# Developer-Zer0/GIF-synthesis-with-Discrete-Diffusion

Hardware: NVIDIA B200
Metric: reverse_step_token_updates_per_sec (higher is better)
Workload: dtype f32

## Files before the change

gif-synthesis-with-discrete-diffusion_b200/csrc/d3pm_ptx.cuh:

```cuda
#pragma once

#include <cuda_runtime.h>
#include <stdint.h>

namespace d3pm {

__device__ __forceinline__ uint32_t smem_u32(const void* p) { return static_cast<uint32_t>(__cvta_generic_to_shared(p)); }

__device__ __forceinline__ void mbar_init(unsigned long long* bar, uint32_t count) {
  asm volatile("mbarrier.init.shared::cta.b64 [%0], %1;" ::"r"(smem_u32(bar)), "r"(count) : "memory");
}
__device__ __forceinline__ void fence_mbarrier_init() { asm volatile("fence.mbarrier_init.release.cluster;" ::: "memory"); }
__device__ __forceinline__ void mbar_expect_tx(unsigned long long* bar, uint32_t bytes) {
  asm volatile("mbarrier.arrive.expect_tx.shared::cta.b64 _, [%0], %1;" ::"r"(smem_u32(bar)), "r"(bytes) : "memory");
}
__device__ __forceinline__ void mbar_arrive(unsigned long long* bar) {
  asm volatile("mbarrier.arrive.shared::cta.b64 _, [%0];" ::"r"(smem_u32(bar)) : "memory");
}
__device__ __forceinline__ void mbar_arrive_remote(unsigned long long* bar, uint32_t cta) {
  uint32_t r;
  asm volatile("mapa.shared::cluster.u32 %0, %1, %2;" : "=r"(r) : "r"(smem_u32(bar)), "r"(cta));
  asm volatile("mbarrier.arrive.release.cluster.shared::cluster.b64 _, [%0];" ::"r"(r) : "memory");
}
__device__ __forceinline__ bool mbar_test(unsigned long long* bar, uint32_t parity) {
  uint32_t done;
  asm volatile(
      "{\n\t.reg .pred p;\n\t"
      "mbarrier.test_wait.parity.shared::cta.b64 p, [%1], %2;\n\t"
      "selp.u32 %0, 1, 0, p;\n\t}"
      : "=r"(done)
      : "r"(smem_u32(bar)), "r"(parity)
      : "memory");
  return done != 0;
}
__device__ __forceinline__ void mbar_wait(unsigned long long* bar, uint32_t parity) {
  asm volatile(
      "{\n\t.reg .pred p;\n\t"
      "WAIT_%=:\n\t"
      "mbarrier.try_wait.parity.shared::cta.b64 p, [%0], %1, %2;\n\t"
      "@p bra DONE_%=;\n\t"
      "bra WAIT_%=;\n\t"
      "DONE_%=:\n\t}"
      ::"r"(smem_u32(bar)), "r"(parity), "r"(0x989680)
      : "memory");
}
__device__ __forceinline__ void mbar_wait_spin(unsigned long long* bar, uint32_t parity) {
  const uint32_t addr = smem_u32(bar);
  uint32_t done;
  do {
    asm volatile(
        "{\n\t.reg .pred p;\n\t"
        "mbarrier.try_wait.parity.shared::cta.b64 p, [%1], %2;\n\t"
        "selp.u32 %0, 1, 0, p;\n\t}"
        : "=r"(done)
        : "r"(addr), "r"(parity)
        : "memory");
  } while (!done);
}
__device__ __forceinline__ void mbar_wait_cluster(unsigned long long* bar, uint32_t parity) {
  asm volatile(
      "{\n\t.reg .pred p;\n\t"
      "WAIT_%=:\n\t"
      "mbarrier.try_wait.parity.acquire.cluster.shared::cta.b64 p, [%0], %1, %2;\n\t"
      "@p bra DONE_%=;\n\t"
      "bra WAIT_%=;\n\t"
      "DONE_%=:\n\t}"
      ::"r"(smem_u32(bar)), "r"(parity), "r"(0x989680)
      : "memory");
}

__device__ __forceinline__ void tma_load(void* dst, const void* src, uint32_t bytes, unsigned long long* bar) {
  asm volatile(
      "cp.async.bulk.shared::cluster.global.mbarrier::complete_tx::bytes [%0], [%1], %2, [%3];"
      ::"r"(smem_u32(dst)), "l"(src), "r"(bytes), "r"(smem_u32(bar))
      : "memory");
}
__device__ __forceinline__ void fence_proxy_async() { asm volatile("fence.proxy.async.shared::cta;" ::: "memory"); }

__device__ __forceinline__ void tc_fence_before() { asm volatile("tcgen05.fence::before_thread_sync;" ::: "memory"); }
__device__ __forceinline__ void tc_fence_after() { asm volatile("tcgen05.fence::after_thread_sync;" ::: "memory"); }
__device__ __forceinline__ void tc_commit(unsigned long long* bar) {
  asm volatile("tcgen05.commit.cta_group::1.mbarrier::arrive::one.shared::cluster.b64 [%0];" ::"r"(smem_u32(bar)) : "memory");
}
__device__ __forceinline__ void tc_commit_pair(unsigned long long* bar) {
  asm volatile("tcgen05.commit.cta_group::2.mbarrier::arrive::one.shared::cluster.multicast::cluster.b64 [%0], %1;" ::"r"(smem_u32(bar)),
               "h"(static_cast<unsigned short>(3))
               : "memory");
}
constexpr uint32_t idesc_tf32(int M, int N) {
  return (1u << 4) | (2u << 7) | (2u << 10) | ((static_cast<uint32_t>(N) >> 3) << 17) | ((static_cast<uint32_t>(M) >> 4) << 24);
}
__device__ __forceinline__ void tc_mma_tf32(uint32_t d_tmem, uint64_t a_desc, uint64_t b_desc, uint32_t idesc, uint32_t accumulate) {
  asm volatile(
      "{\n\t.reg .pred p;\n\t"
      "setp.ne.b32 p, %4, 0;\n\t"
      "tcgen05.mma.cta_group::1.kind::tf32 [%0], %1, %2, %3, p;\n\t}"
      ::"r"(d_tmem), "l"(a_desc), "l"(b_desc), "r"(idesc), "r"(accumulate)
      : "memory");
}
__device__ __forceinline__ void tc_mma_tf32_pair(uint32_t d_tmem, uint64_t a_desc, uint64_t b_desc, uint32_t idesc, uint32_t accumulate) {
  asm volatile(
      "{\n\t.reg .pred p;\n\t"
      "setp.ne.b32 p, %4, 0;\n\t"
      "tcgen05.mma.cta_group::2.kind::tf32 [%0], %1, %2, %3, p;\n\t}"
      ::"r"(d_tmem), "l"(a_desc), "l"(b_desc), "r"(idesc), "r"(accumulate)
      : "memory");
}
__device__ __forceinline__ uint64_t smem_desc(uint32_t addr) {
  return static_cast<uint64_t>((addr >> 4) & 0x3fffu) | (static_cast<uint64_t>(1024 >> 4) << 32) | (1ull << 46) | (2ull << 61);
}

template <int CTAS, int NCOLS>
__device__ __forceinline__ void tmem_alloc(uint32_t* slot) {
  static_assert(CTAS == 1 || CTAS == 2, "cta_group::1 or ::2");
  if constexpr (CTAS == 2)
    asm volatile("tcgen05.alloc.cta_group::2.sync.aligned.shared::cta.b32 [%0], %1;" ::"r"(smem_u32(slot)), "n"(NCOLS) : "memory");
  else
    asm volatile("tcgen05.alloc.cta_group::1.sync.aligned.shared::cta.b32 [%0], %1;" ::"r"(smem_u32(slot)), "n"(NCOLS) : "memory");
}
template <int CTAS>
__device__ __forceinline__ void tmem_relinquish() {
  static_assert(CTAS == 1 || CTAS == 2, "cta_group::1 or ::2");
  if constexpr (CTAS == 2) asm volatile("tcgen05.relinquish_alloc_permit.cta_group::2.sync.aligned;" ::: "memory");
  else asm volatile("tcgen05.relinquish_alloc_permit.cta_group::1.sync.aligned;" ::: "memory");
}
template <int CTAS, int NCOLS>
__device__ __forceinline__ void tmem_dealloc(uint32_t taddr) {
  static_assert(CTAS == 1 || CTAS == 2, "cta_group::1 or ::2");
  if constexpr (CTAS == 2) asm volatile("tcgen05.dealloc.cta_group::2.sync.aligned.b32 %0, %1;" ::"r"(taddr), "n"(NCOLS) : "memory");
  else asm volatile("tcgen05.dealloc.cta_group::1.sync.aligned.b32 %0, %1;" ::"r"(taddr), "n"(NCOLS) : "memory");
}
__device__ __forceinline__ void tmem_ld16(uint32_t taddr, uint32_t (&v)[16]) {
  asm volatile(
      "tcgen05.ld.sync.aligned.32x32b.x16.b32 "
      "{%0, %1, %2, %3, %4, %5, %6, %7, %8, %9, %10, %11, %12, %13, %14, %15}, [%16];"
      : "=r"(v[0]), "=r"(v[1]), "=r"(v[2]), "=r"(v[3]), "=r"(v[4]), "=r"(v[5]), "=r"(v[6]), "=r"(v[7]), "=r"(v[8]),
        "=r"(v[9]), "=r"(v[10]), "=r"(v[11]), "=r"(v[12]), "=r"(v[13]), "=r"(v[14]), "=r"(v[15])
      : "r"(taddr)
      : "memory");
}
__device__ __forceinline__ void tmem_ld32(uint32_t taddr, uint32_t (&v)[32]) {
  asm volatile(
      "tcgen05.ld.sync.aligned.32x32b.x32.b32 "
      "{%0, %1, %2, %3, %4, %5, %6, %7, %8, %9, %10, %11, %12, %13, %14, %15, "
      "%16, %17, %18, %19, %20, %21, %22, %23, %24, %25, %26, %27, %28, %29, %30, %31}, [%32];"
      : "=r"(v[0]), "=r"(v[1]), "=r"(v[2]), "=r"(v[3]), "=r"(v[4]), "=r"(v[5]), "=r"(v[6]), "=r"(v[7]), "=r"(v[8]),
        "=r"(v[9]), "=r"(v[10]), "=r"(v[11]), "=r"(v[12]), "=r"(v[13]), "=r"(v[14]), "=r"(v[15]), "=r"(v[16]),
        "=r"(v[17]), "=r"(v[18]), "=r"(v[19]), "=r"(v[20]), "=r"(v[21]), "=r"(v[22]), "=r"(v[23]), "=r"(v[24]),
        "=r"(v[25]), "=r"(v[26]), "=r"(v[27]), "=r"(v[28]), "=r"(v[29]), "=r"(v[30]), "=r"(v[31])
      : "r"(taddr)
      : "memory");
}
__device__ __forceinline__ void tmem_ld_wait() { asm volatile("tcgen05.wait::ld.sync.aligned;" ::: "memory"); }

__device__ __forceinline__ uint32_t cluster_ctarank() {
  uint32_t r;
  asm volatile("mov.u32 %0, %%cluster_ctarank;" : "=r"(r));
  return r;
}
__device__ __forceinline__ void cluster_sync() {
  asm volatile("barrier.cluster.arrive.release;" ::: "memory");
  asm volatile("barrier.cluster.wait.acquire;" ::: "memory");
}

}
```

gif-synthesis-with-discrete-diffusion_b200/csrc/d3pm_step_stream.cuh:

```cuda
#pragma once

#include <type_traits>

#include "d3pm_host.h"
#include "d3pm_ptx.cuh"
#include "d3pm_step_rows.cuh"
#include "d3pm_stream.cuh"

namespace d3pm {

constexpr int kCandPerRow = 30;
constexpr float kStreamThin = 8.0f;
constexpr float kRedoThin = 16.0f;
struct RowInfo {
  float A, Bc, Pj, PK, accept;
  uint32_t j;
  int32_t rel;
  int32_t pad;
};

template <int NP, int CPT, bool HAS_U>
struct StreamShape {
  static_assert(CPT == 8 || (CPT == 16 && !HAS_U), "64 classes per thread only fit in registers without the second tensor");
  static constexpr int K = 1024 * NP;
  static constexpr int GT = 256 * NP / CPT;
  static constexpr int NW = GT / 32;
  static constexpr int NG = kStreamThreads / GT;
  static constexpr int SB = 128 / NG;
  static constexpr int RC = 8192 / NG;
  static constexpr int PS = 128 / GT;
  static constexpr int NCALL = CPT / 2;
  static_assert(GT >= 32 && GT <= 128 && NG <= 16, "unsupported group shape");
};

template <int NP, int CPT, bool HAS_U>
struct __align__(128) GroupSmem {
  using Sh = StreamShape<NP, CPT, HAS_U>;
  float c[1024 * NP];
  float u[HAS_U ? 1024 * NP : 4];
  alignas(16) float red[3][6 * 4];
  unsigned long long full;
  unsigned long long keys[4];
  uint32_t redo_cnt;
  uint32_t pad;
  RowInfo info[Sh::SB];
  uint32_t cand_cnt[Sh::SB];
  uint32_t cand_k[Sh::SB][kCandPerRow];
  float cand_p[Sh::SB][kCandPerRow];
  int32_t redo[Sh::RC];
};

template <int NW, int NV, typename Sync>
__device__ __forceinline__ void stream_max_sum(float (&m)[NV], float (&s)[NV], float* scratch, Sync sync) {
  const int lane = threadIdx.x & 31, warp = (threadIdx.x >> 5) & (NW - 1);
#pragma unroll
  for (int v = 0; v < NV; ++v) {
    const float mw = warp_max(m[v]);
    const float mw2 = to_log2_units(mw);
    const float sw = warp_sum(s[v] * ex2(to_log2_units(m[v]) - mw2));
    if (NW == 1) {
      m[v] = mw, s[v] = sw;
    } else if (lane == 0) {
      scratch[(3 * v) * 4 + warp] = mw;
      scratch[(3 * v + 1) * 4 + warp] = mw2;
      scratch[(3 * v + 2) * 4 + warp] = sw;
    }
  }
  sync();
  if constexpr (NW > 1) {
#pragma unroll
  for (int v = 0; v < NV; ++v) {
    const float4 mw = lds_warps<NW>(scratch + (3 * v) * 4, -CUDART_INF_F), mw2 = lds_warps<NW>(scratch + (3 * v + 1) * 4, 0.f);
    const float4 sw = lds_warps<NW>(scratch + (3 * v + 2) * 4, 0.f);
    if (NW == 4) {
      const float M = fmaxf(fmaxf(mw.x, mw.y), fmaxf(mw.z, mw.w));
      const float M2 = to_log2_units(M);
      m[v] = M;
      s[v] = fmaf(sw.x, ex2(mw2.x - M2), fmaf(sw.y, ex2(mw2.y - M2), fmaf(sw.z, ex2(mw2.z - M2), sw.w * ex2(mw2.w - M2))));
    } else {
      const float M = fmaxf(mw.x, mw.y);
      const float M2 = to_log2_units(M);
      m[v] = M;
      s[v] = fmaf(sw.x, ex2(mw2.x - M2), sw.y * ex2(mw2.y - M2));
    }
  }
  }
}

template <int NW, int NV, typename Sync>
__device__ __forceinline__ void stream_max(float* mx, float* scratch, Sync sync) {
  const int lane = threadIdx.x & 31, warp = (threadIdx.x >> 5) & (NW - 1);
#pragma unroll
  for (int v = 0; v < NV; ++v) {
    const float a = warp_max(mx[v]);
    if (NW == 1) mx[v] = a;
    else if (lane == 0) scratch[v * 4 + warp] = a;
  }
  sync();
  if constexpr (NW > 1) {
#pragma unroll
  for (int v = 0; v < NV; ++v) {
    const float4 a = lds_warps<NW>(scratch + v * 4, -CUDART_INF_F);
    mx[v] = fmaxf(fmaxf(a.x, a.y), fmaxf(a.z, a.w));
  }
  }
}

template <int NW, int NV, typename Sync>
__device__ __forceinline__ void stream_sum(float (&s)[NV], float* scratch, Sync sync) {
  const int lane = threadIdx.x & 31, warp = (threadIdx.x >> 5) & (NW - 1);
#pragma unroll
  for (int v = 0; v < NV; ++v) {
    const float sw = warp_sum(s[v]);
    if (NW == 1) s[v] = sw;
    else if (lane == 0) scratch[v * 4 + warp] = sw;
  }
  sync();
  if constexpr (NW > 1) {
#pragma unroll
  for (int v = 0; v < NV; ++v) {
    const float4 a = lds_warps<NW>(scratch + v * 4, 0.f);
    s[v] = (a.x + a.y) + (a.z + a.w);
  }
  }
}

template <int NW, typename Sync>
__device__ __forceinline__ unsigned long long stream_max_u64(unsigned long long key, unsigned long long* scratch, Sync sync) {
  const int lane = threadIdx.x & 31, warp = (threadIdx.x >> 5) & (NW - 1);
  key = warp_max_u64(key);
  if (NW == 1) {
    sync();
    return key;
  }
  if (lane == 0) scratch[warp] = key;
  sync();
  unsigned long long best = scratch[0];
#pragma unroll
  for (int w = 1; w < NW; ++w) best = scratch[w] > best ? scratch[w] : best;
  return best;
}

template <int NP, int CPT, bool HAS_U>
__device__ __noinline__ void score_batch(GroupSmem<NP, CPT, HAS_U>& S, int nslots, const ParamNoiseStream& rng, const StepParams& p, int G,
                                         int first_row) {
  using Sh = StreamShape<NP, CPT, HAS_U>;
  constexpr uint32_t K = 1024u * NP;
  const int lane = threadIdx.x & 31, warp = (threadIdx.x >> 5) & (Sh::NW - 1);
  const int sub = lane & 15;
  for (int slot = 2 * warp + (lane >> 4); slot - (lane >> 4) < nslots; slot += 2 * Sh::NW) {
    unsigned long long key = 0ull;
    float lp = 0.f;
    const bool live = slot < nslots;
    RowInfo ri;
    ri.accept = 0.f, ri.rel = 0;
    uint32_t cnt = 0;
    if (live) {
      ri = S.info[slot];
      cnt = S.cand_cnt[slot];
      const uint32_t n = cnt < static_cast<uint32_t>(kCandPerRow) ? cnt : static_cast<uint32_t>(kCandPerRow);
      const uint64_t grow = static_cast<uint64_t>(p.row_offset + (first_row + ri.rel * G));
      for (uint32_t item = static_cast<uint32_t>(sub); item < n + 2u; item += 16u) {
        uint32_t k = 0;
        float P = 0.f;
        bool have = false;
        if (item < n) {
          k = S.cand_k[slot][item];
          const float pe = fminf(fmaxf(S.cand_p[slot][item], kPFloor), 1.0f);
          P = fmaf(pe, ri.A, ri.Bc);
          have = (k != ri.j);
        } else if (item == n) {
          k = K, P = ri.PK, have = true;
        } else if (ri.j != K) {
          k = ri.j, P = ri.Pj, have = true;
        }
        if (have) {
          const float lpk = log_prob_clamped(P);
          const float sc = lpk + gumbel_from_uniform(uniform_from_draw(rng.draw(k, grow)));
          const unsigned long long kk = pack_key(sc, k);
          if (kk > key) key = kk, lp = lpk;
        }
      }
    }
    const unsigned long long mine = key;
#pragma unroll
    for (int o = 8; o > 0; o >>= 1) {
      const unsigned long long other = __shfl_xor_sync(0xffffffffu, key, o);
      key = other > key ? other : key;
    }
    const bool accepted = live && cnt <= static_cast<uint32_t>(kCandPerRow) && key_score(key) >= ri.accept;
    if (live && sub == 0) {
      if (accepted) {
        p.x_prev[first_row + ri.rel * G] = key_class(key);
      } else {
        S.redo[atomicAdd(&S.redo_cnt, 1u)] = ri.rel;
      }
      S.cand_cnt[slot] = 0;
    }
    if (p.winner_post != nullptr && accepted && mine == key && mine != 0ull) p.winner_post[first_row + ri.rel * G] = lp;
  }
}

template <int NP, int CPT, bool HAS_U, bool RECON, int LD = D3PM_LOGITS_F32>
__global__ void __launch_bounds__(kStreamThreads, 1) step_stream_kernel(const __grid_constant__ StepParams p) {
  extern __shared__ __align__(128) unsigned char smem_raw[];
  using Sh = StreamShape<NP, CPT, HAS_U>;
  using Smem = GroupSmem<NP, CPT, HAS_U>;
  constexpr int K = Sh::K, GT = Sh::GT, NW = Sh::NW, NG = Sh::NG, PS = Sh::PS, NCALL = Sh::NCALL;
  constexpr int NC = CPT;
  using LT = LogitType<LD>;
  constexpr uint32_t kRowBytes = K * LT::kBytes;
  uint32_t tid;
  asm volatile("mov.u32 %0, %%tid.x;" : "=r"(tid));
  const int g = tid / GT;
  const int tg = tid % GT;
  Smem& S = reinterpret_cast<Smem*>(smem_raw)[g];
  const StreamSync<NW> sync{g + 1};
  const int G = static_cast<int>(gridDim.x) * NG;
  const int first_row = g * static_cast<int>(gridDim.x) + static_cast<int>(blockIdx.x);
  const int rows = static_cast<int>(p.rows);
  const uint32_t pitch = static_cast<uint32_t>(p.pitch_logits);
  const bool exact_mode = (p.sample_mode == D3PM_SAMPLE_PHILOX_EXACT);
  if (tg == 0) {
    mbar_init(&S.full, 1);
    fence_mbarrier_init();
    S.redo_cnt = 0;
    if (!exact_mode && first_row < rows) {
      const unsigned long long at = static_cast<unsigned long long>(static_cast<uint32_t>(first_row)) * pitch;
      mbar_expect_tx(&S.full, HAS_U ? 2 * kRowBytes : kRowBytes);
      tma_load(S.c, LT::row(p.logits_c, at), kRowBytes, &S.full);
      if (HAS_U) tma_load(S.u, LT::row(p.logits_u, at), kRowBytes, &S.full);
    }
  }
  float* coef_s = reinterpret_cast<float*>(smem_raw + sizeof(Smem) * NG);
  const bool coef_in_smem = p.T <= kCoefSmemRows;
  if (coef_in_smem) {
    for (int i = tid; i < p.T * 16; i += kStreamThreads)
      coef_s[i] = __ldg(p.coef_table + static_cast<size_t>(i >> 4) * D3PM_COEF_STRIDE + (i & 15));
  }
  const ParamNoiseStream rng(NoiseKeysParam(p.keys), p.offset);
  const float thin_c = p.thin_factor > 0.f ? p.thin_factor : kStreamThin;
  for (int i = tg; i < Sh::SB; i += GT) S.cand_cnt[i] = 0;
  __syncthreads();

  auto issue_row = [&](int row) {
    const unsigned long long at = static_cast<unsigned long long>(static_cast<uint32_t>(row)) * pitch;
    fence_proxy_async();
    mbar_expect_tx(&S.full, HAS_U ? 2 * kRowBytes : kRowBytes);
    tma_load(S.c, LT::row(p.logits_c, at), kRowBytes, &S.full);
    if (HAS_U) tma_load(S.u, LT::row(p.logits_u, at), kRowBytes, &S.full);
  };
  auto slot_lo = [](int c) { return (c / PS) * 2 * PS + (c % PS); };

  uint32_t phase = 0;
  uint32_t status_bits = 0;
#ifdef D3PM_STREAM_TIMING
  auto now_ns = [] { unsigned long long v; asm volatile("mov.u64 %0, %%globaltimer;" : "=l"(v)); return v; };
  const unsigned long long tm_start = now_ns();
  unsigned long long tm_main = 0;
  uint32_t tm_rows = 0, tm_redo = 0;
#endif

  auto process_row = [&](auto exact_c, int row, int next_row, uint32_t j, int tt, int slot, int rel) {
    constexpr bool exact = decltype(exact_c)::value;
    const bool masked = (j == static_cast<uint32_t>(K));
    mbar_wait_spin(&S.full, phase);
    phase ^= 1u;

    float2 x[NC][2], z[HAS_U ? NC : 1][2];
#pragma unroll
    for (int i = 0; i < NC; ++i) {
      const int q = GT * i + tg;
      LT::chunk(S.c, q, x[i][0], x[i][1]);
      if (HAS_U) LT::chunk(S.u, q, z[i][0], z[i][1]);
    }
    auto e_of = [&](int i, int h) -> float2& {
      if constexpr (HAS_U) return z[i][h];
      else return x[i][h];
    };
    const float xj = masked ? 0.f : LT::one(S.c, j);
    const float zj = (HAS_U && !masked) ? LT::one(S.u, j) : 0.f;

    float am[2] = {0.f, 0.f};
    if (HAS_U) {
      am[0] = fmaxf(fmaxf(fabsf(x[0][0].x), fabsf(x[0][0].y)), fmaxf(fabsf(x[0][1].x), fabsf(x[0][1].y)));
      am[1] = fmaxf(fmaxf(fabsf(z[0][0].x), fabsf(z[0][0].y)), fmaxf(fabsf(z[0][1].x), fabsf(z[0][1].y)));
    }
#pragma unroll
    for (int i = 1; i < NC; ++i) {
      if (HAS_U)
        am[0] = fmaxf(fmaxf(am[0], fabsf(x[i][0].x)), fmaxf(fabsf(x[i][0].y), fmaxf(fabsf(x[i][1].x), fabsf(x[i][1].y))));
      if (HAS_U)
        am[1] = fmaxf(fmaxf(am[1], fabsf(z[i][0].x)), fmaxf(fabsf(z[i][0].y), fmaxf(fabsf(z[i][1].x), fabsf(z[i][1].y))));
    }
    if (HAS_U) stream_max<NW, 2>(am, S.red[0], sync);
    else sync();
    if (!exact && tg == 0 && next_row >= 0) issue_row(next_row);

    const uint64_t grow = static_cast<uint64_t>(p.row_offset + row);

    float My2, rSy, r, yj;
    const float2 l2e = make_float2(kLog2e, kLog2e);
    if (HAS_U) {
      const float gs = p.guidance_scale, og = 1.0f - gs;
      const float2 gs2 = make_float2(gs, gs), og2 = make_float2(og, og);
      float my = -CUDART_INF_F;
      constexpr float kLnK = NP == 4 ? 8.3178f : (NP == 2 ? 7.6247f : 6.9315f);
      constexpr float kSafeAbs = 0.5f * (69.99f - kLnK);
      const bool no_clamp = (am[0] <= kSafeAbs) && (am[1] <= kSafeAbs) && (fabsf(gs) * am[0] + fabsf(og) * am[1] <= 160.0f);
      if (no_clamp) {
#pragma unroll
        for (int i = 0; i < NC; ++i)
#pragma unroll
          for (int h = 0; h < 2; ++h) {
            const float2 y = __ffma2_rn(gs2, x[i][h], __fmul2_rn(og2, z[i][h]));
            x[i][h] = y;
            my = fmaxf(my, fmaxf(y.x, y.y));
          }
        yj = fmaf(gs, xj, og * zj);
      } else {
        float mx[2], s[2];
        mx[0] = fmaxf(fmaxf(x[0][0].x, x[0][0].y), fmaxf(x[0][1].x, x[0][1].y));
        mx[1] = fmaxf(fmaxf(z[0][0].x, z[0][0].y), fmaxf(z[0][1].x, z[0][1].y));
#pragma unroll
        for (int i = 1; i < NC; ++i) {
          mx[0] = fmaxf(fmaxf(mx[0], x[i][0].x), fmaxf(x[i][0].y, fmaxf(x[i][1].x, x[i][1].y)));
          mx[1] = fmaxf(fmaxf(mx[1], z[i][0].x), fmaxf(z[i][0].y, fmaxf(z[i][1].x, z[i][1].y)));
        }
        stream_max<NW, 2>(mx, S.red[2], sync);
        mx[0] = fmaxf(mx[0], -3.0e38f), mx[1] = fmaxf(mx[1], -3.0e38f);
        {
          const float mc2 = to_log2_units(mx[0]), mu2 = to_log2_units(mx[1]);
          const float2 nmc = make_float2(-mc2, -mc2), nmu = make_float2(-mu2, -mu2);
          float2 sc[2] = {make_float2(0.f, 0.f), make_float2(0.f, 0.f)}, su[2] = {sc[0], sc[0]};
#pragma unroll
          for (int i = 0; i < NC; ++i)
#pragma unroll
            for (int h = 0; h < 2; ++h) {
              const float2 ac = __ffma2_rn(x[i][h], l2e, nmc), au = __ffma2_rn(z[i][h], l2e, nmu);
              sc[h] = __fadd2_rn(sc[h], make_float2(ex2(ac.x), ex2(ac.y)));
              su[h] = __fadd2_rn(su[h], make_float2(ex2(au.x), ex2(au.y)));
            }
          s[0] = (sc[0].x + sc[0].y) + (sc[1].x + sc[1].y);
          s[1] = (su[0].x + su[0].y) + (su[1].x + su[1].y);
        }
        stream_sum<NW, 2>(s, S.red[2] + 2 * 4, sync);
        const float lnSc = ln_rel_sum(mx[0], s[0]), lnSu = ln_rel_sum(mx[1], s[1]);
        const float ta = kClampLo + lnSc, tb = kClampLo + lnSu;
        const float C = fmaf(-gs, lnSc, -og * lnSu);
        const float2 nMc = make_float2(-mx[0], -mx[0]), nMu = make_float2(-mx[1], -mx[1]), C2 = make_float2(C, C);
#pragma unroll
        for (int i = 0; i < NC; ++i)
#pragma unroll
          for (int h = 0; h < 2; ++h) {
            float2 a = __fadd2_rn(x[i][h], nMc), b = __fadd2_rn(z[i][h], nMu);
            a.x = fmaxf(a.x, ta), a.y = fmaxf(a.y, ta);
            b.x = fmaxf(b.x, tb), b.y = fmaxf(b.y, tb);
            const float2 y = __ffma2_rn(gs2, a, __ffma2_rn(og2, b, C2));
            x[i][h] = y;
            my = fmaxf(my, fmaxf(y.x, y.y));
          }
        yj = fmaf(gs, fmaxf(xj - mx[0], ta), fmaf(og, fmaxf(zj - mx[1], tb), C));
      }
      const float my2 = to_log2_units(my);
      {
        const float2 nmy = make_float2(-my2, -my2);
        float2 sy[2] = {make_float2(0.f, 0.f), make_float2(0.f, 0.f)};
#pragma unroll
        for (int i = 0; i < NC; ++i)
#pragma unroll
          for (int h = 0; h < 2; ++h) {
            const float2 ay = __ffma2_rn(x[i][h], l2e, nmy);
            const float2 ey = make_float2(ex2(ay.x), ex2(ay.y));
            e_of(i, h) = ey;
            sy[h] = __fadd2_rn(sy[h], ey);
          }
        float mm[1] = {my}, ss[1] = {(sy[0].x + sy[0].y) + (sy[1].x + sy[1].y)};
        stream_max_sum<NW, 1>(mm, ss, S.red[1], sync);
        My2 = to_log2_units(mm[0]);
        rSy = __fdividef(1.0f, ss[0]);
      }
      r = ex2(my2 - My2) * rSy;
    } else {
      float mx[1];
      mx[0] = fmaxf(fmaxf(x[0][0].x, x[0][0].y), fmaxf(x[0][1].x, x[0][1].y));
#pragma unroll
      for (int i = 1; i < NC; ++i) mx[0] = fmaxf(fmaxf(mx[0], x[i][0].x), fmaxf(x[i][0].y, fmaxf(x[i][1].x, x[i][1].y)));
      mx[0] = fmaxf(mx[0], -3.0e38f);
      const float mc2 = to_log2_units(mx[0]);
      const float2 nmc = make_float2(-mc2, -mc2);
      float2 sc[2] = {make_float2(0.f, 0.f), make_float2(0.f, 0.f)};
#pragma unroll
      for (int i = 0; i < NC; ++i)
#pragma unroll
        for (int h = 0; h < 2; ++h) {
          const float2 ac = __ffma2_rn(x[i][h], l2e, nmc);
          const float2 ec = make_float2(ex2(ac.x), ex2(ac.y));
          e_of(i, h) = ec;
          sc[h] = __fadd2_rn(sc[h], ec);
        }
      float ss[1] = {(sc[0].x + sc[0].y) + (sc[1].x + sc[1].y)};
      stream_max_sum<NW, 1>(mx, ss, S.red[1], sync);
      My2 = to_log2_units(mx[0]);
      rSy = __fdividef(1.0f, ss[0]);
      r = ex2(mc2 - My2) * rSy;
      yj = xj;
    }
    const float pj = masked ? 0.f : fminf(fmaxf(ex2(fmaf(yj, kLog2e, -My2)) * rSy, kPFloor), 1.0f);
    RowCoef cf;
    if (coef_in_smem) {
      const float* crow = coef_s + tt * 16 + (masked ? 0 : 8);
      cf = row_coef_from(lds4(crow), lds4(crow + 4), masked);
    } else {
      cf = load_row_coef(p.coef_table, tt, masked);
    }
    RowMath rm;
    if (RECON) {
      rm.init_recon(masked ? 0.f : pj, masked ? static_cast<uint32_t>(K) + 1u : j);
      if (tg == 0 && p.score != nullptr) p.score[row] = fminf(fmaxf(rSy, kPFloor), 1.0f);
    } else {
      rm.init(cf, masked, pj, j, K);
    }

    if constexpr (!exact) {
      const ThinRule thin(rm, thin_c);
      const float thrA = r * thin.scaleA, nthrB = -thin.thrB;
      const float2 tA2 = make_float2(thrA, thrA);
      if (tg == 0) {
        RowInfo ri;
        ri.A = rm.A, ri.Bc = rm.Bc, ri.Pj = rm.Pj, ri.PK = rm.PK, ri.accept = thin.accept;
        ri.j = j, ri.rel = rel, ri.pad = 0;
        S.info[slot] = ri;
      }
#pragma unroll
      for (int c0 = 0; c0 < NCALL; c0 += 4) {
        uint4 cws[4];
#pragma unroll
        for (int c = 0; c < 4; ++c) cws[c] = rng.coarse(ParamNoiseStream::coarse_call_of_chunk(GT * slot_lo(c0 + c) + tg), grow);
#pragma unroll
        for (int c = 0; c < 4; ++c) {
          const int lo = slot_lo(c0 + c);
          const uint32_t w4[4] = {cws[c].x, cws[c].y, cws[c].z, cws[c].w};
          float slack = -4.0f;
#pragma unroll
          for (int w = 0; w < 4; ++w) {
            const float2 nf = make_float2(__uint_as_float(__byte_perm(w4[w], 0xbf80u, 0x5410)),
                                          __uint_as_float(__byte_perm(w4[w], 0xbf80u, 0x5432)));
            const float2 d = __ffma2_rn(e_of(lo + (w >> 1) * PS, w & 1), tA2, nf);
            slack = fmaxf(slack, fmaxf(d.x, d.y));
          }
          if (slack >= nthrB) {
#pragma unroll
            for (int w = 0; w < 4; ++w)
#pragma unroll
              for (int hl = 0; hl < 2; ++hl) {
                const float2 ee = e_of(lo + (w >> 1) * PS, w & 1);
                const float e = hl ? ee.y : ee.x;
                const uint32_t h16 = hl ? (w4[w] >> 16) : (w4[w] & 0xffffu);
                const float nf = __uint_as_float(0xbf800000u | h16);
                if (fmaf(e, thrA, nf) >= nthrB) {
                  const uint32_t pos = atomicAdd(&S.cand_cnt[slot], 1u);
                  if (pos < static_cast<uint32_t>(kCandPerRow)) {
                    S.cand_k[slot][pos] = 4u * (GT * (lo + (w >> 1) * PS) + tg) + 2u * (w & 1) + hl;
                    S.cand_p[slot][pos] = e * r;
                  }
                }
              }
          }
        }
      }
      return;
    } else {
    unsigned long long best = 0ull;
    float best_lp = 0.f;
    bool settled = false;
    if (!exact_mode) {
      const ThinRule thin2(rm, (p.thin_factor > 0.f && p.thin_factor < 0.01f) ? p.thin_factor : kRedoThin);
      const float thrA = r * thin2.scaleA;
      const float2 tA2 = make_float2(thrA, thrA), tB2 = make_float2(thin2.thrB, thin2.thrB);
#pragma unroll
      for (int c = 0; c < NCALL; ++c) {
        const int lo = slot_lo(c);
        const uint4 cw = rng.coarse(ParamNoiseStream::coarse_call_of_chunk(GT * lo + tg), grow);
        const uint32_t w4[4] = {cw.x, cw.y, cw.z, cw.w};
        uint32_t hits = 0;
        float ev[8];
#pragma unroll
        for (int w = 0; w < 4; ++w) {
          const float2 ee = e_of(lo + (w >> 1) * PS, w & 1);
          ev[2 * w] = ee.x, ev[2 * w + 1] = ee.y;
          const float2 nf = make_float2(__uint_as_float(__byte_perm(w4[w], 0xbf80u, 0x5410)),
                                        __uint_as_float(__byte_perm(w4[w], 0xbf80u, 0x5432)));
          const float2 d = __ffma2_rn(ee, tA2, __fadd2_rn(tB2, nf));
          hits |= (d.x >= 0.0f ? 1u : 0u) << (2 * w);
          hits |= (d.y >= 0.0f ? 1u : 0u) << (2 * w + 1);
        }
        while (hits != 0) {
          const int b = __ffs(hits) - 1;
          hits &= hits - 1;
          float e = 0.f;
#pragma unroll
          for (int q = 0; q < 8; ++q) e = (b == q) ? ev[q] : e;
          const uint32_t k = 4u * (GT * (lo + (b >> 2) * PS) + tg) + static_cast<uint32_t>(b & 3);
          if (k != j) {
            const float lpk = rm.post_of(k, e, r);
            const unsigned long long key = pack_key(lpk + gumbel_from_uniform(uniform_from_draw(rng.draw(k, grow))), k);
            if (key > best) best = key, best_lp = lpk;
          }
        }
      }
      if (tg == 0) {
        const float lpk = rm.post_mask();
        const unsigned long long key = pack_key(lpk + gumbel_from_uniform(uniform_from_draw(rng.draw(K, grow))), K);
        if (key > best) best = key, best_lp = lpk;
      }
      if (tg == GT - 1 && !masked) {
        const float lpk = rm.post_self();
        const unsigned long long key = pack_key(lpk + gumbel_from_uniform(uniform_from_draw(rng.draw(j, grow))), j);
        if (key > best) best = key, best_lp = lpk;
      }
      const unsigned long long mine = best;
      best = stream_max_u64<NW>(best, S.keys, sync);
      settled = key_score(best) >= thin2.accept;
      if (settled) {
        if (p.winner_post != nullptr && mine == best) p.winner_post[row] = best_lp;
      } else {
        best = 0ull;
        sync();
      }
    }
    if (!settled) {
#pragma unroll
      for (int i = 0; i < NC; ++i) {
        const float2 a = e_of(i, 0), b = e_of(i, 1);
        *reinterpret_cast<float4*>(S.c + 4 * (GT * i + tg)) = make_float4(a.x, a.y, b.x, b.y);
      }
#pragma unroll 1
      for (int i = 0; i < NC; ++i) {
        const uint32_t q = static_cast<uint32_t>(GT) * i + tg;
        const float4 e4 = lds4(S.c + 4 * q);
        const float ev[4] = {e4.x, e4.y, e4.z, e4.w};
        const uint4 cw = rng.coarse(ParamNoiseStream::coarse_call_of_chunk(q), grow);
        const uint4 fw = rng.fine(q >> 2, grow);
#pragma unroll
        for (int e = 0; e < 4; ++e) {
          const uint32_t k = 4u * q + e;
          const uint32_t mdraw =
              (ParamNoiseStream::half_of(cw, (((q >> 7) & 1u) << 2) | e) << 7) | ParamNoiseStream::low7_of(fw, ((q & 3u) << 2) | e);
          const float lpk = rm.post_of(k, ev[e], r);
          const unsigned long long key = pack_key(lpk + gumbel_from_uniform(uniform_from_draw(mdraw)), k);
          if (key > best) best = key, best_lp = lpk;
        }
      }
      if (tg == 0) {
        const float lpk = rm.post_mask();
        const unsigned long long key = pack_key(lpk + gumbel_from_uniform(uniform_from_draw(rng.draw(K, grow))), K);
        if (key > best) best = key, best_lp = lpk;
      }
      const unsigned long long mine = best;
      best = stream_max_u64<NW>(best, S.keys, sync);
      if (p.winner_post != nullptr && mine == best) p.winner_post[row] = best_lp;
    }
    if (tg == 0) {
      p.x_prev[row] = key_class(best);
      if (next_row >= 0) issue_row(next_row);
    }
    }
  };

  const int N = p.N;
  auto token_of = [&](int r_) { return static_cast<long long>(p.x_t[r_]); };
  auto time_of = [&](int b_) { return static_cast<long long>(p.t[b_]); };
  auto checked = [&](long long tt, long long jj, int& t_cur, uint32_t& j_cur) {
    if (static_cast<unsigned long long>(tt) >= static_cast<unsigned long long>(p.T)) {
      status_bits |= D3PM_STATUS_BAD_T;
      tt = tt < 0 ? 0 : p.T - 1;
    }
    if (static_cast<unsigned long long>(jj) > static_cast<unsigned long long>(K)) {
      status_bits |= D3PM_STATUS_BAD_TOKEN;
      jj = K;
    }
    t_cur = static_cast<int>(tt), j_cur = static_cast<uint32_t>(jj);
    asm volatile("" : "+r"(t_cur), "+r"(j_cur) : : "memory");
  };
  if (!exact_mode) {
    const int stepB = G / N, stepR = G % N;
    int vb = first_row / N, vr = first_row % N;
    int row = first_row < rows ? first_row : -1;
    long long jj = 0, tt = 0;
    if (row >= 0) {
      jj = token_of(row);
      tt = time_of(vb);
    }
    int it = 0, in_batch = 0;
    while (row >= 0) {
      int t_cur;
      uint32_t j_cur;
      checked(tt, jj, t_cur, j_cur);
      const int next = row + G < rows ? row + G : -1;
      vb += stepB, vr += stepR;
      if (vr >= N) vr -= N, ++vb;
      if (next >= 0) {
        jj = token_of(next);
        tt = time_of(vb);
      }
      process_row(std::false_type{}, row, next, j_cur, t_cur, in_batch, it);
#ifdef D3PM_STREAM_TIMING
      ++tm_rows;
#endif
      row = next;
      ++it;
      if (++in_batch == Sh::SB || row < 0) {
        sync();
        score_batch<NP, CPT, HAS_U>(S, in_batch, rng, p, G, first_row);
        sync();
        in_batch = 0;
      }
    }
  }
#ifdef D3PM_STREAM_TIMING
  tm_main = now_ns();
#endif
  {
    const uint32_t n2 = exact_mode ? (first_row < rows ? static_cast<uint32_t>((rows - first_row + G - 1) / G) : 0u) : S.redo_cnt;
    auto row_at = [&](uint32_t i) { return first_row + (exact_mode ? static_cast<int>(i) : S.redo[i]) * G; };
    if (n2 > 0) {
      if (!exact_mode) status_bits |= D3PM_STATUS_FALLBACK;
      int row = row_at(0);
      if (tg == 0) issue_row(row);
      long long jj = token_of(row), tt = time_of(row / N);
      for (uint32_t i = 0; i < n2; ++i) {
        int t_cur;
        uint32_t j_cur;
        checked(tt, jj, t_cur, j_cur);
        const int next = (i + 1 < n2) ? row_at(i + 1) : -1;
        if (next >= 0) {
          jj = token_of(next);
          tt = time_of(next / N);
        }
        process_row(std::true_type{}, row, next, j_cur, t_cur, 0, 0);
#ifdef D3PM_STREAM_TIMING
        ++tm_redo;
#endif
        row = next;
      }
    }
  }
#ifdef D3PM_STREAM_TIMING
  if (tg == 0 && p.status != nullptr) {
    const unsigned long long tm_end = now_ns();
    uint32_t* o = p.status + 8 * (blockIdx.x * NG + g);
    uint32_t smid;
    asm volatile("mov.u32 %0, %%smid;" : "=r"(smid));
    o[0] = static_cast<uint32_t>(tm_start), o[1] = static_cast<uint32_t>(tm_start >> 32);
    o[2] = static_cast<uint32_t>(tm_main - tm_start), o[3] = static_cast<uint32_t>(tm_end - tm_start);
    o[4] = tm_rows, o[5] = tm_redo, o[6] = smid, o[7] = 0;
  }
#else
  if (status_bits != 0 && tg == 0 && p.status != nullptr) atomicOr(p.status, status_bits);
#endif
}

constexpr long long kStreamMinRows = 1024;

inline bool stream_kernel_supports(const StepParams& p) {
  if (p.sample_mode != D3PM_SAMPLE_PHILOX && p.sample_mode != D3PM_SAMPLE_PHILOX_EXACT) return false;
  if (p.post != nullptr || p.recon != nullptr || p.gap != nullptr || p.x_prev == nullptr) return false;
  if (p.sharpen != nullptr || (p.score != nullptr && p.sample_from != D3PM_FROM_RECON)) return false;
  if (p.K != 1024 && p.K != 2048 && p.K != 4096) return false;
  if (p.pitch_logits >= (1LL << 32)) return false;
  if (p.logits_dtype != D3PM_LOGITS_F32 && (p.sample_from == D3PM_FROM_RECON || p.pitch_logits % 8 != 0)) return false;
  return true;
}

inline long long stream_kernel_max_rows() { return 8192LL * host::sm_count(); }

template <int NP, int CPT, bool HAS_U>
int launch_step_stream_t(const StepParams& p, cudaStream_t s) {
  const size_t smem = sizeof(GroupSmem<NP, CPT, HAS_U>) * StreamShape<NP, CPT, HAS_U>::NG + kCoefSmemRows * 16 * sizeof(float);
  const bool recon = p.sample_from == D3PM_FROM_RECON;
  if (p.logits_dtype == D3PM_LOGITS_F16)
    return recon ? D3PM_ERR_UNSUPPORTED : launch_persistent(step_stream_kernel<NP, CPT, HAS_U, false, D3PM_LOGITS_F16>, kStreamThreads, smem, p, s);
  if (p.logits_dtype == D3PM_LOGITS_BF16)
    return recon ? D3PM_ERR_UNSUPPORTED : launch_persistent(step_stream_kernel<NP, CPT, HAS_U, false, D3PM_LOGITS_BF16>, kStreamThreads, smem, p, s);
  return launch_persistent(recon ? step_stream_kernel<NP, CPT, HAS_U, true> : step_stream_kernel<NP, CPT, HAS_U, false>,
                           kStreamThreads, smem, p, s);
}

inline int launch_step_stream(const StepParams& p, cudaStream_t s) {
  const bool has_u = p.logits_u != nullptr;
  switch (p.K) {
    case 1024: return has_u ? launch_step_stream_t<1, 8, true>(p, s) : launch_step_stream_t<1, 8, false>(p, s);
    case 2048: return has_u ? launch_step_stream_t<2, 8, true>(p, s) : launch_step_stream_t<2, 16, false>(p, s);
    case 4096: return has_u ? launch_step_stream_t<4, 8, true>(p, s) : launch_step_stream_t<4, 16, false>(p, s);
    default: return D3PM_ERR_UNSUPPORTED;
  }
}

}
```

gif-synthesis-with-discrete-diffusion_b200/csrc/d3pm_stream.cuh:

```cuda
#pragma once

#include <cuda_bf16.h>
#include <cuda_fp16.h>

#include <type_traits>

#include "d3pm_common.cuh"
#include "d3pm_host.h"

namespace d3pm {

constexpr int kStreamThreads = 512;
constexpr int kCoefSmemRows = 256;

template <int NW>
struct StreamSync {
  int id;
  __device__ __forceinline__ void operator()() const {
    if (NW == 1) __syncwarp();
    else asm volatile("bar.sync %0, %1;" ::"r"(id), "n"(32 * NW) : "memory");
  }
};
__device__ __forceinline__ float4 lds4(const float* p) { return *reinterpret_cast<const float4*>(p); }
template <int LD>
struct LogitType {
  static constexpr uint32_t kBytes = LD == D3PM_LOGITS_F32 ? 4u : 2u;
  static __device__ __forceinline__ float2 widen(uint32_t pair) {
    if constexpr (LD == D3PM_LOGITS_BF16) {
      return make_float2(__uint_as_float(pair << 16), __uint_as_float(pair & 0xffff0000u));
    } else {
      return __half22float2(*reinterpret_cast<const __half2*>(&pair));
    }
  }
  static __device__ __forceinline__ void chunk(const float* stage, int q, float2& lo, float2& hi) {
    if constexpr (LD == D3PM_LOGITS_F32) {
      const float4 a = lds4(stage + 4 * q);
      lo = make_float2(a.x, a.y), hi = make_float2(a.z, a.w);
    } else {
      const uint2 raw = *reinterpret_cast<const uint2*>(reinterpret_cast<const unsigned char*>(stage) + 8 * q);
      lo = widen(raw.x), hi = widen(raw.y);
    }
  }
  static __device__ __forceinline__ float one(const float* stage, uint32_t k) {
    if constexpr (LD == D3PM_LOGITS_F32) {
      return stage[k];
    } else {
      const uint32_t h = reinterpret_cast<const unsigned short*>(stage)[k];
      if constexpr (LD == D3PM_LOGITS_BF16) return __uint_as_float(h << 16);
      else return __half2float(__ushort_as_half(static_cast<unsigned short>(h)));
    }
  }
  static __device__ __forceinline__ const void* row(const float* base, unsigned long long elements) {
    return reinterpret_cast<const unsigned char*>(base) + elements * kBytes;
  }
  using Elem = std::conditional_t<LD == D3PM_LOGITS_F32, float, unsigned short>;
  static __device__ __forceinline__ uint32_t narrow2(float lo, float hi) {
    uint32_t bits;
    if constexpr (LD == D3PM_LOGITS_BF16) {
      const __nv_bfloat162 v = __float22bfloat162_rn(make_float2(lo, hi));
      bits = *reinterpret_cast<const uint32_t*>(&v);
    } else {
      const __half2 v = __float22half2_rn(make_float2(lo, hi));
      bits = *reinterpret_cast<const uint32_t*>(&v);
    }
    return bits;
  }
  static __device__ __forceinline__ Elem narrow1(float v) {
    if constexpr (LD == D3PM_LOGITS_F32) return v;
    else if constexpr (LD == D3PM_LOGITS_BF16) return __bfloat16_as_ushort(__float2bfloat16_rn(v));
    else return __half_as_ushort(__float2half_rn(v));
  }
  static __device__ __forceinline__ void store4(Elem* rowp, uint32_t q, const float (&o)[4]) {
    if constexpr (LD == D3PM_LOGITS_F32) {
      st_stream4(rowp + 4 * q, make_float4(o[0], o[1], o[2], o[3]));
    } else {
      st_stream_b64(rowp + 4 * q, narrow2(o[0], o[1]), narrow2(o[2], o[3]));
    }
  }
};
template <int NW>
__device__ __forceinline__ float4 lds_warps(const float* p, float neutral) {
  if (NW == 4) return lds4(p);
  const float2 a = *reinterpret_cast<const float2*>(p);
  return make_float4(a.x, a.y, neutral, neutral);
}

__device__ __forceinline__ float warp_min(float x) {
  float m;
  asm volatile("redux.sync.min.f32 %0, %1, 0xffffffff;" : "=f"(m) : "f"(x));
  return m;
}

template <typename Params>
int launch_persistent(void (*kern)(Params), int threads, size_t smem, const Params& p, cudaStream_t s) {
  const int sms = host::sm_count();
  if (sms == 0) return D3PM_ERR_CUDA;
  if (cudaFuncSetAttribute(kern, cudaFuncAttributeMaxDynamicSharedMemorySize, static_cast<int>(smem)) != cudaSuccess)
    return D3PM_ERR_CUDA;
  kern<<<static_cast<unsigned>(sms), threads, smem, s>>>(p);
  return D3PM_OK;
}

}
```

Measured before the change: 204.3 million.

## Double-buffer survivor lists, interleave scoring, add L2 prefetch and PDL launch

Splits the per-row candidate lists into two buffers so scoring of the previous batch is interleaved with streaming the next rows, replacing the batch-boundary sync-and-score stall. Adds L2 bulk prefetch of upcoming logits rows, switches the redo list to a bitmap, and launches with programmatic dependent launch (griddepcontrol) so consecutive step kernels overlap their prologues. Doubles the survivor-list shared memory and adds more complex scheduling logic. It also adds timing instrumentation behind a macro.

Measured after the change: 205.4 million, median of 6. Within noise of the previous version (+0.6%).

```diff
diff --git a/gif-synthesis-with-discrete-diffusion_b200/csrc/d3pm_ptx.cuh b/gif-synthesis-with-discrete-diffusion_b200/csrc/d3pm_ptx.cuh
--- a/gif-synthesis-with-discrete-diffusion_b200/csrc/d3pm_ptx.cuh
+++ b/gif-synthesis-with-discrete-diffusion_b200/csrc/d3pm_ptx.cuh
@@ -75,7 +75,13 @@
       ::"r"(smem_u32(dst)), "l"(src), "r"(bytes), "r"(smem_u32(bar))
       : "memory");
 }
+__device__ __forceinline__ void prefetch_l2(const void* src, uint32_t bytes) {
+  asm volatile("cp.async.bulk.prefetch.L2.global [%0], %1;" ::"l"(src), "r"(bytes) : "memory");
+}
 __device__ __forceinline__ void fence_proxy_async() { asm volatile("fence.proxy.async.shared::cta;" ::: "memory"); }
+
+__device__ __forceinline__ void griddep_wait() { asm volatile("griddepcontrol.wait;" ::: "memory"); }
+__device__ __forceinline__ void griddep_launch_dependents() { asm volatile("griddepcontrol.launch_dependents;" ::: "memory"); }
 
 __device__ __forceinline__ void tc_fence_before() { asm volatile("tcgen05.fence::before_thread_sync;" ::: "memory"); }
 __device__ __forceinline__ void tc_fence_after() { asm volatile("tcgen05.fence::after_thread_sync;" ::: "memory"); }
diff --git a/gif-synthesis-with-discrete-diffusion_b200/csrc/d3pm_step_stream.cuh b/gif-synthesis-with-discrete-diffusion_b200/csrc/d3pm_step_stream.cuh
--- a/gif-synthesis-with-discrete-diffusion_b200/csrc/d3pm_step_stream.cuh
+++ b/gif-synthesis-with-discrete-diffusion_b200/csrc/d3pm_step_stream.cuh
@@ -7,6 +7,12 @@
 #include "d3pm_step_rows.cuh"
 #include "d3pm_stream.cuh"
 
+#ifndef D3PM_L2_AHEAD
+#define D3PM_L2_AHEAD 1
+#endif
+#ifndef D3PM_STEP_PDL
+#define D3PM_STEP_PDL true
+#endif
 namespace d3pm {
 
 constexpr int kCandPerRow = 30;
@@ -33,6 +39,14 @@
   static_assert(GT >= 32 && GT <= 128 && NG <= 16, "unsupported group shape");
 };
 
+template <int SB>
+struct SurvivorLists {
+  RowInfo info[SB];
+  uint32_t cnt[SB];
+  uint32_t k[SB][kCandPerRow];
+  float p[SB][kCandPerRow];
+};
+
 template <int NP, int CPT, bool HAS_U>
 struct __align__(128) GroupSmem {
   using Sh = StreamShape<NP, CPT, HAS_U>;
@@ -43,11 +57,8 @@
   unsigned long long keys[4];
   uint32_t redo_cnt;
   uint32_t pad;
-  RowInfo info[Sh::SB];
-  uint32_t cand_cnt[Sh::SB];
-  uint32_t cand_k[Sh::SB][kCandPerRow];
-  float cand_p[Sh::SB][kCandPerRow];
-  int32_t redo[Sh::RC];
+  SurvivorLists<Sh::SB> lists[2];
+  uint32_t redo[Sh::RC / 32];
 };
 
 template <int NW, int NV, typename Sync>
@@ -142,22 +153,22 @@
 }
 
 template <int NP, int CPT, bool HAS_U>
-__device__ __noinline__ void score_batch(GroupSmem<NP, CPT, HAS_U>& S, int nslots, const ParamNoiseStream& rng, const StepParams& p, int G,
-                                         int first_row) {
+__device__ __noinline__ void score_batch(GroupSmem<NP, CPT, HAS_U>& S, SurvivorLists<StreamShape<NP, CPT, HAS_U>::SB>& L, int s0,
+                                         int s1, const ParamNoiseStream& rng, const StepParams& p, int G, int first_row) {
   using Sh = StreamShape<NP, CPT, HAS_U>;
   constexpr uint32_t K = 1024u * NP;
   const int lane = threadIdx.x & 31, warp = (threadIdx.x >> 5) & (Sh::NW - 1);
   const int sub = lane & 15;
-  for (int slot = 2 * warp + (lane >> 4); slot - (lane >> 4) < nslots; slot += 2 * Sh::NW) {
+  for (int slot = s0 + 2 * warp + (lane >> 4); slot - (lane >> 4) < s1; slot += 2 * Sh::NW) {
     unsigned long long key = 0ull;
     float lp = 0.f;
-    const bool live = slot < nslots;
+    const bool live = slot < s1;
     RowInfo ri;
     ri.accept = 0.f, ri.rel = 0;
     uint32_t cnt = 0;
     if (live) {
-      ri = S.info[slot];
-      cnt = S.cand_cnt[slot];
+      ri = L.info[slot];
+      cnt = L.cnt[slot];
       const uint32_t n = cnt < static_cast<uint32_t>(kCandPerRow) ? cnt : static_cast<uint32_t>(kCandPerRow);
       const uint64_t grow = static_cast<uint64_t>(p.row_offset + (first_row + ri.rel * G));
       for (uint32_t item = static_cast<uint32_t>(sub); item < n + 2u; item += 16u) {
@@ -165,8 +176,8 @@
         float P = 0.f;
         bool have = false;
         if (item < n) {
-          k = S.cand_k[slot][item];
-          const float pe = fminf(fmaxf(S.cand_p[slot][item], kPFloor), 1.0f);
+          k = L.k[slot][item];
+          const float pe = fminf(fmaxf(L.p[slot][item], kPFloor), 1.0f);
           P = fmaf(pe, ri.A, ri.Bc);
           have = (k != ri.j);
         } else if (item == n) {
@@ -193,9 +204,10 @@
       if (accepted) {
         p.x_prev[first_row + ri.rel * G] = key_class(key);
       } else {
-        S.redo[atomicAdd(&S.redo_cnt, 1u)] = ri.rel;
-      }
-      S.cand_cnt[slot] = 0;
+        atomicOr(&S.redo[ri.rel >> 5], 1u << (ri.rel & 31));
+        atomicAdd(&S.redo_cnt, 1u);
+      }
+      L.cnt[slot] = 0;
     }
     if (p.winner_post != nullptr && accepted && mine == key && mine != 0ull) p.winner_post[first_row + ri.rel * G] = lp;
   }
@@ -225,12 +237,28 @@
     mbar_init(&S.full, 1);
     fence_mbarrier_init();
     S.redo_cnt = 0;
-    if (!exact_mode && first_row < rows) {
-      const unsigned long long at = static_cast<unsigned long long>(static_cast<uint32_t>(first_row)) * pitch;
-      mbar_expect_tx(&S.full, HAS_U ? 2 * kRowBytes : kRowBytes);
-      tma_load(S.c, LT::row(p.logits_c, at), kRowBytes, &S.full);
-      if (HAS_U) tma_load(S.u, LT::row(p.logits_u, at), kRowBytes, &S.full);
-    }
+  }
+  for (int i = tg; i < 2 * Sh::SB; i += GT) S.lists[i / Sh::SB].cnt[i % Sh::SB] = 0;
+  for (int i = tg; i < Sh::RC / 32; i += GT) S.redo[i] = 0;
+  const ParamNoiseStream rng(NoiseKeysParam(p.keys), p.offset);
+  const float thin_c = p.thin_factor > 0.f ? p.thin_factor : kStreamThin;
+  auto prefetch_ahead = [&](int row) {
+#pragma unroll
+    for (int a = 1; a <= D3PM_L2_AHEAD; ++a) {
+      const int ahead = row + a * G;
+      if (ahead >= rows) break;
+      const unsigned long long at = static_cast<unsigned long long>(static_cast<uint32_t>(ahead)) * pitch;
+      prefetch_l2(LT::row(p.logits_c, at), kRowBytes);
+      if (HAS_U) prefetch_l2(LT::row(p.logits_u, at), kRowBytes);
+    }
+  };
+  griddep_wait();
+  if (tg == 0 && !exact_mode && first_row < rows) {
+    const unsigned long long at = static_cast<unsigned long long>(static_cast<uint32_t>(first_row)) * pitch;
+    mbar_expect_tx(&S.full, HAS_U ? 2 * kRowBytes : kRowBytes);
+    tma_load(S.c, LT::row(p.logits_c, at), kRowBytes, &S.full);
+    if (HAS_U) tma_load(S.u, LT::row(p.logits_u, at), kRowBytes, &S.full);
+    prefetch_ahead(first_row);
   }
   float* coef_s = reinterpret_cast<float*>(smem_raw + sizeof(Smem) * NG);
   const bool coef_in_smem = p.T <= kCoefSmemRows;
@@ -238,9 +266,6 @@
     for (int i = tid; i < p.T * 16; i += kStreamThreads)
       coef_s[i] = __ldg(p.coef_table + static_cast<size_t>(i >> 4) * D3PM_COEF_STRIDE + (i & 15));
   }
-  const ParamNoiseStream rng(NoiseKeysParam(p.keys), p.offset);
-  const float thin_c = p.thin_factor > 0.f ? p.thin_factor : kStreamThin;
-  for (int i = tg; i < Sh::SB; i += GT) S.cand_cnt[i] = 0;
   __syncthreads();
 
   auto issue_row = [&](int row) {
@@ -257,14 +282,28 @@
 #ifdef D3PM_STREAM_TIMING
   auto now_ns = [] { unsigned long long v; asm volatile("mov.u64 %0, %%globaltimer;" : "=l"(v)); return v; };
   const unsigned long long tm_start = now_ns();
-  unsigned long long tm_main = 0;
+  const long long cy_start = clock64();
+  unsigned long long tm_main = 0, tm_first = 0;
   uint32_t tm_rows = 0, tm_redo = 0;
+  long long cy_wait = 0, cy_score = 0, cy_last = 0;
+#define D3PM_TIMED(acc, ...)           \
+  do {                                 \
+    const long long t0_ = clock64();   \
+    __VA_ARGS__;                       \
+    acc += clock64() - t0_;            \
+  } while (0)
+#else
+#define D3PM_TIMED(acc, ...) __VA_ARGS__
 #endif
 
-  auto process_row = [&](auto exact_c, int row, int next_row, uint32_t j, int tt, int slot, int rel) {
+  auto process_row = [&](auto exact_c, int row, int next_row, uint32_t j, int tt, SurvivorLists<Sh::SB>* L, int slot, int rel) {
     constexpr bool exact = decltype(exact_c)::value;
     const bool masked = (j == static_cast<uint32_t>(K));
-    mbar_wait_spin(&S.full, phase);
+    if constexpr (exact) mbar_wait_spin(&S.full, phase);
+    else D3PM_TIMED(cy_wait, mbar_wait_spin(&S.full, phase));
+#ifdef D3PM_STREAM_TIMING
+    if (tm_first == 0) tm_first = now_ns() - tm_start;
+#endif
     phase ^= 1u;
 
     float2 x[NC][2], z[HAS_U ? NC : 1][2];
@@ -295,7 +334,10 @@
     }
     if (HAS_U) stream_max<NW, 2>(am, S.red[0], sync);
     else sync();
-    if (!exact && tg == 0 && next_row >= 0) issue_row(next_row);
+    if (!exact && tg == 0 && next_row >= 0) {
+      issue_row(next_row);
+      prefetch_ahead(next_row);
+    }
 
     const uint64_t grow = static_cast<uint64_t>(p.row_offset + row);
 
@@ -430,7 +472,7 @@
         RowInfo ri;
         ri.A = rm.A, ri.Bc = rm.Bc, ri.Pj = rm.Pj, ri.PK = rm.PK, ri.accept = thin.accept;
         ri.j = j, ri.rel = rel, ri.pad = 0;
-        S.info[slot] = ri;
+        L->info[slot] = ri;
       }
 #pragma unroll
       for (int c0 = 0; c0 < NCALL; c0 += 4) {
@@ -459,10 +501,10 @@
                 const uint32_t h16 = hl ? (w4[w] >> 16) : (w4[w] & 0xffffu);
                 const float nf = __uint_as_float(0xbf800000u | h16);
                 if (fmaf(e, thrA, nf) >= nthrB) {
-                  const uint32_t pos = atomicAdd(&S.cand_cnt[slot], 1u);
+                  const uint32_t pos = atomicAdd(&L->cnt[slot], 1u);
                   if (pos < static_cast<uint32_t>(kCandPerRow)) {
-                    S.cand_k[slot][pos] = 4u * (GT * (lo + (w >> 1) * PS) + tg) + 2u * (w & 1) + hl;
-                    S.cand_p[slot][pos] = e * r;
+                    L->k[slot][pos] = 4u * (GT * (lo + (w >> 1) * PS) + tg) + 2u * (w & 1) + hl;
+                    L->p[slot][pos] = e * r;
                   }
                 }
               }
@@ -583,6 +625,7 @@
     t_cur = static_cast<int>(tt), j_cur = static_cast<uint32_t>(jj);
     asm volatile("" : "+r"(t_cur), "+r"(j_cur) : : "memory");
   };
+  const int n_mine = first_row < rows ? (rows - first_row + G - 1) / G : 0;
   if (!exact_mode) {
     const int stepB = G / N, stepR = G % N;
     int vb = first_row / N, vr = first_row % N;
@@ -592,7 +635,9 @@
       jj = token_of(row);
       tt = time_of(vb);
     }
-    int it = 0, in_batch = 0;
+    constexpr int kPass = (HAS_U && LD == D3PM_LOGITS_F32) ? 2 * NW : Sh::SB;
+    int it = 0, in_batch = 0, cur = 0;
+    int scored = Sh::SB;
     while (row >= 0) {
       int t_cur;
       uint32_t j_cur;
@@ -604,41 +649,53 @@
         jj = token_of(next);
         tt = time_of(vb);
       }
-      process_row(std::false_type{}, row, next, j_cur, t_cur, in_batch, it);
+      if (scored < Sh::SB && in_batch >= 1 && (in_batch % kPass == 1 || (Sh::SB - scored) / kPass >= n_mine - it)) {
+        D3PM_TIMED(cy_score, score_batch<NP, CPT, HAS_U>(S, S.lists[cur ^ 1], scored, scored + kPass, rng, p, G, first_row));
+        scored += kPass;
+      }
+      if (next < 0) griddep_launch_dependents();
+      process_row(std::false_type{}, row, next, j_cur, t_cur, &S.lists[cur], in_batch, it);
 #ifdef D3PM_STREAM_TIMING
       ++tm_rows;
 #endif
       row = next;
       ++it;
-      if (++in_batch == Sh::SB || row < 0) {
-        sync();
-        score_batch<NP, CPT, HAS_U>(S, in_batch, rng, p, G, first_row);
-        sync();
-        in_batch = 0;
-      }
-    }
+      if (++in_batch == Sh::SB) in_batch = 0, cur ^= 1, scored = 0;
+    }
+    D3PM_TIMED(cy_last, sync();
+               if (scored < Sh::SB) score_batch<NP, CPT, HAS_U>(S, S.lists[cur ^ 1], scored, Sh::SB, rng, p, G, first_row);
+               if (in_batch > 0) score_batch<NP, CPT, HAS_U>(S, S.lists[cur], 0, in_batch, rng, p, G, first_row);
+               sync());
   }
 #ifdef D3PM_STREAM_TIMING
   tm_main = now_ns();
 #endif
   {
-    const uint32_t n2 = exact_mode ? (first_row < rows ? static_cast<uint32_t>((rows - first_row + G - 1) / G) : 0u) : S.redo_cnt;
-    auto row_at = [&](uint32_t i) { return first_row + (exact_mode ? static_cast<int>(i) : S.redo[i]) * G; };
-    if (n2 > 0) {
+    auto next_rel = [&](int from) -> int {
+      if (exact_mode) return from < n_mine ? from : -1;
+      for (int w = from >> 5; w < (n_mine + 31) >> 5; ++w) {
+        const uint32_t bits = S.redo[w] & (w == (from >> 5) ? ~0u << (from & 31) : ~0u);
+        if (bits != 0) return 32 * w + __ffs(bits) - 1;
+      }
+      return -1;
+    };
+    int rel = (exact_mode || S.redo_cnt != 0) ? next_rel(0) : -1;
+    if (rel >= 0) {
       if (!exact_mode) status_bits |= D3PM_STATUS_FALLBACK;
-      int row = row_at(0);
+      int row = first_row + rel * G;
       if (tg == 0) issue_row(row);
       long long jj = token_of(row), tt = time_of(row / N);
-      for (uint32_t i = 0; i < n2; ++i) {
+      while (row >= 0) {
         int t_cur;
         uint32_t j_cur;
         checked(tt, jj, t_cur, j_cur);
-        const int next = (i + 1 < n2) ? row_at(i + 1) : -1;
+        rel = next_rel(rel + 1);
+        const int next = rel >= 0 ? first_row + rel * G : -1;
         if (next >= 0) {
           jj = token_of(next);
           tt = time_of(next / N);
         }
-        process_row(std::true_type{}, row, next, j_cur, t_cur, 0, 0);
+        process_row(std::true_type{}, row, next, j_cur, t_cur, nullptr, 0, 0);
 #ifdef D3PM_STREAM_TIMING
         ++tm_redo;
 #endif
@@ -649,16 +706,20 @@
 #ifdef D3PM_STREAM_TIMING
   if (tg == 0 && p.status != nullptr) {
     const unsigned long long tm_end = now_ns();
-    uint32_t* o = p.status + 8 * (blockIdx.x * NG + g);
+    uint32_t* o = p.status + 16 * (blockIdx.x * NG + g);
     uint32_t smid;
     asm volatile("mov.u32 %0, %%smid;" : "=r"(smid));
     o[0] = static_cast<uint32_t>(tm_start), o[1] = static_cast<uint32_t>(tm_start >> 32);
     o[2] = static_cast<uint32_t>(tm_main - tm_start), o[3] = static_cast<uint32_t>(tm_end - tm_start);
-    o[4] = tm_rows, o[5] = tm_redo, o[6] = smid, o[7] = 0;
+    o[4] = tm_rows, o[5] = tm_redo, o[6] = smid, o[7] = static_cast<uint32_t>(tm_first);
+    o[8] = static_cast<uint32_t>(clock64() - cy_start), o[9] = static_cast<uint32_t>(cy_wait);
+    o[10] = static_cast<uint32_t>(cy_score), o[11] = static_cast<uint32_t>(cy_last);
+    o[12] = o[13] = o[14] = o[15] = 0;
   }
 #else
   if (status_bits != 0 && tg == 0 && p.status != nullptr) atomicOr(p.status, status_bits);
 #endif
+#undef D3PM_TIMED
 }
 
 constexpr long long kStreamMinRows = 1024;
@@ -680,11 +741,13 @@
   const size_t smem = sizeof(GroupSmem<NP, CPT, HAS_U>) * StreamShape<NP, CPT, HAS_U>::NG + kCoefSmemRows * 16 * sizeof(float);
   const bool recon = p.sample_from == D3PM_FROM_RECON;
   if (p.logits_dtype == D3PM_LOGITS_F16)
-    return recon ? D3PM_ERR_UNSUPPORTED : launch_persistent(step_stream_kernel<NP, CPT, HAS_U, false, D3PM_LOGITS_F16>, kStreamThreads, smem, p, s);
+    return recon ? D3PM_ERR_UNSUPPORTED
+                 : launch_persistent(step_stream_kernel<NP, CPT, HAS_U, false, D3PM_LOGITS_F16>, kStreamThreads, smem, p, s, D3PM_STEP_PDL);
   if (p.logits_dtype == D3PM_LOGITS_BF16)
-    return recon ? D3PM_ERR_UNSUPPORTED : launch_persistent(step_stream_kernel<NP, CPT, HAS_U, false, D3PM_LOGITS_BF16>, kStreamThreads, smem, p, s);
+    return recon ? D3PM_ERR_UNSUPPORTED
+                 : launch_persistent(step_stream_kernel<NP, CPT, HAS_U, false, D3PM_LOGITS_BF16>, kStreamThreads, smem, p, s, D3PM_STEP_PDL);
   return launch_persistent(recon ? step_stream_kernel<NP, CPT, HAS_U, true> : step_stream_kernel<NP, CPT, HAS_U, false>,
-                           kStreamThreads, smem, p, s);
+                           kStreamThreads, smem, p, s, D3PM_STEP_PDL);
 }
 
 inline int launch_step_stream(const StepParams& p, cudaStream_t s) {
diff --git a/gif-synthesis-with-discrete-diffusion_b200/csrc/d3pm_stream.cuh b/gif-synthesis-with-discrete-diffusion_b200/csrc/d3pm_stream.cuh
--- a/gif-synthesis-with-discrete-diffusion_b200/csrc/d3pm_stream.cuh
+++ b/gif-synthesis-with-discrete-diffusion_b200/csrc/d3pm_stream.cuh
@@ -92,13 +92,26 @@
 }
 
 template <typename Params>
-int launch_persistent(void (*kern)(Params), int threads, size_t smem, const Params& p, cudaStream_t s) {
+int launch_persistent(void (*kern)(Params), int threads, size_t smem, const Params& p, cudaStream_t s, bool programmatic = false) {
   const int sms = host::sm_count();
   if (sms == 0) return D3PM_ERR_CUDA;
   if (cudaFuncSetAttribute(kern, cudaFuncAttributeMaxDynamicSharedMemorySize, static_cast<int>(smem)) != cudaSuccess)
     return D3PM_ERR_CUDA;
-  kern<<<static_cast<unsigned>(sms), threads, smem, s>>>(p);
-  return D3PM_OK;
+  if (!programmatic) {
+    kern<<<static_cast<unsigned>(sms), threads, smem, s>>>(p);
+    return D3PM_OK;
+  }
+  cudaLaunchAttribute attr;
+  attr.id = cudaLaunchAttributeProgrammaticStreamSerialization;
+  attr.val.programmaticStreamSerializationAllowed = 1;
+  cudaLaunchConfig_t cfg = {};
+  cfg.gridDim = dim3(static_cast<unsigned>(sms));
+  cfg.blockDim = dim3(static_cast<unsigned>(threads));
+  cfg.dynamicSmemBytes = smem;
+  cfg.stream = s;
+  cfg.attrs = &attr;
+  cfg.numAttrs = 1;
+  return cudaLaunchKernelEx(&cfg, kern, p) == cudaSuccess ? D3PM_OK : D3PM_ERR_CUDA;
 }
 
 }
```
